# xmengli/H-DenseUNet

Measured on AMD Instinct MI355X. Metric: CT slices/sec fwd+bwd (2D 512^2), higher is better.
Workload: dtype bf16

## Files before the change

### h-denseunet_amd/csrc/conv_common.h

```cpp
#pragma once
#include "hdu_platform.h"

struct ConvK {
  const void* x;
  const void* skip;
  const void* w;
  void* y;
  const float* pro_a;
  const float* pro_b;
  const float* bias;
  const float* epi_a;
  const float* epi_b;
  int epi_relu;
  long long ldx, ldskip, ldy;
  long long M;
  int N, Di, Hi, Wi, Cin;
  int De, He, We;
  int ud, uh, uw;
  int KD, KH, KW, sd, sh, sw, pd, ph, pw;
  int Do, Ho, Wo, Cout;
  int Ktot;
  unsigned div_wo_mul, div_wo_shr, div_ho_mul, div_ho_shr, div_do_mul, div_do_shr;
  unsigned spread_h, spread_d;
  unsigned div_cin_mul, div_cin_shr, div_kw_mul, div_kw_shr, div_kh_mul, div_kh_shr;
  unsigned x_bytes, w_bytes;
  unsigned sk_div_mul, sk_div_shr;
  int pro_relu, accumulate;
  float drop_scale;
  unsigned drop_thresh;
  unsigned drop_seed;
  const unsigned* drop_seed_dev;
  int xcd_swizzle;
  int wg_gx, wg_gy, wg_gz;
  int debug_flags;
  int vec_out;
  int f32_split;
  float* stats_partial;
  const float* stats_shift;
  int stats_slots;
  const void* bnb_u; long long bnb_ldu;
  const float* bnb_a; const float* bnb_b; const float* bnb_mean; const float* bnb_rstd;
  float* bnb_partial; int bnb_slots; int bnb_relu;
  float* sk_ws;
  unsigned* sk_cnt;
  long long M_layer;
};

__device__ __forceinline__ unsigned hdu_fastdiv(unsigned n, unsigned mul, unsigned shr) {
  return mul == 0u ? n : (unsigned)(((unsigned long long)n * mul) >> 32) >> shr;
}

__device__ __forceinline__ void hdu_k_state(const ConvK& p, int k, int& c, int& kd, int& kh, int& kw, int& tap_i) {
  const unsigned tap = hdu_fastdiv((unsigned)k, p.div_cin_mul, p.div_cin_shr);
  tap_i = (int)tap;
  c = k - (int)tap * p.Cin;
  const unsigned t = hdu_fastdiv(tap, p.div_kw_mul, p.div_kw_shr);
  kw = (int)(tap - t * (unsigned)p.KW);
  const unsigned d = hdu_fastdiv(t, p.div_kh_mul, p.div_kh_shr);
  kh = (int)(t - d * (unsigned)p.KH);
  kd = (int)d;
}

__device__ __forceinline__ unsigned hdu_bit_range(int lo, int hi) {
  return (hi >= 32 ? 0xffffffffu : (1u << hi) - 1u) & ~((1u << lo) - 1u);
}

__device__ __forceinline__ unsigned hdu_tap_range_mask(int i0, int K, int E) {
  const int lo = i0 < 0 ? -i0 : 0;
  const int hi = E - i0 < K ? E - i0 : K;
  return hi > lo ? (hi >= 32 ? 0xffffffffu : (1u << hi) - 1u) & ~((1u << lo) - 1u) : 0u;
}

template <bool FAST>
__device__ __forceinline__ void hdu_row_state(const ConvK& p, unsigned m, bool pointwise, int& rn, int& rid, int& rih, int& riw,
                                              int& rpix, unsigned& rmask) {
  rmask = 0u;
  if (FAST && pointwise) {
// ... 55 lines not shown
```

### h-denseunet_amd/csrc/conv_halo_wide.hip

```cpp
#include "conv_common.h"
#include "hdu_host.h"

typedef float f32x16 __attribute__((ext_vector_type(16)));

__device__ __forceinline__ f32x16 hdu_mfma_32x32x16_bf16(u32x4 a, u32x4 b, f32x16 c) {
#ifdef HDU_EMU
  return hipemu_mfma_32x32x16_bf16(__builtin_bit_cast(hipemu_u16x8, a), __builtin_bit_cast(hipemu_u16x8, b), c);
#else
  return __builtin_amdgcn_mfma_f32_32x32x16_bf16(__builtin_bit_cast(hdu_bf16x8, a), __builtin_bit_cast(hdu_bf16x8, b), c, 0, 0, 0);
#endif
}

template <int N> __device__ __forceinline__ void hw_wait_vmcnt() {
  static_assert(N >= 0 && N < 64, "vmcnt immediate");
#ifndef HDU_EMU
  asm volatile("s_waitcnt vmcnt(%0)" ::"i"(N) : "memory");
#endif
}

template <int TH_, int NT_, int WAVES_M_, int WAVES_N_, int NS_> struct HaloWide {
  static constexpr int TH = TH_, NT = NT_, WAVES_M = WAVES_M_, WAVES_N = WAVES_N_, NS = NS_;
  static constexpr int NW = WAVES_M * WAVES_N, NTHR = NW * 64;
  static constexpr int TW = 32, HC = TW + 2, HR = TH + 2, HP = HR * HC;
  static constexpr int BN = NT * 32, BM = TH * TW;
  static constexpr int XI = (HP * 2 + 63) / 64;
  static constexpr int WI = (BN * 18 + 63) / 64;
  static constexpr int LPW = (XI + WI + NW - 1) / NW;
  static constexpr int STAGE = LPW * NW * 1024;
  static constexpr int XBYTES = XI * 1024;
  static constexpr int ROWB = BN * 2 + 16;
  static constexpr int SMEM = NS * STAGE > BM * ROWB ? NS * STAGE : BM * ROWB;
  static constexpr int MT = TH / WAVES_M, NTW = NT / WAVES_N;
  static_assert(TH % WAVES_M == 0 && NT % WAVES_N == 0, "wave layout");
  static_assert(SMEM <= 160 * 1024, "LDS");
  static_assert((NS - 2) * LPW < 64, "vmcnt");
};

template <typename C, typename RowValid>
__device__ __forceinline__ void hw_epilogue_stats(const ConvK& p, const char* smem, int n0, int tid, unsigned slot, RowValid valid) {
  constexpr int NCC = C::BN / 8, CPI = C::NTHR / 16;
  float* dst = p.stats_partial + (long long)(slot % (unsigned)p.stats_slots) * 2 * p.Cout;
  const int rl = tid & 15;
#pragma unroll 1
  for (int it = 0; it < (NCC + CPI - 1) / CPI; ++it) {
    const int cc = (tid >> 4) + it * CPI;
    const int nbase = n0 + cc * 8;
    const bool col = cc < NCC && nbase < p.Cout;
    const int ccq = col ? cc : 0, nc = col ? nbase : 0;
    float s1[8], s2[8], sh[8];
#pragma unroll
    for (int j = 0; j < 8; j += 4) {
      const f32x4 v4 = *(const f32x4*)(p.stats_shift + nc + j);
      sh[j] = v4[0]; sh[j + 1] = v4[1]; sh[j + 2] = v4[2]; sh[j + 3] = v4[3];
    }
#pragma unroll
    for (int j = 0; j < 8; ++j) { s1[j] = 0.f; s2[j] = 0.f; }
#pragma unroll 1
    for (int q0 = 0; q0 < C::BM / 16; q0 += 8) {
      u32x4 rv[8];
#pragma unroll
      for (int q = 0; q < 8; ++q) rv[q] = *(const u32x4*)(smem + (rl + (q0 + q) * 16) * C::ROWB + ccq * 16);
#pragma unroll
      for (int q = 0; q < 8; ++q) {
        const float keep = (col && valid(rl + (q0 + q) * 16)) ? 1.f : 0.f;
        float f[8];
        Chunk<bf16_t>::unpack(rv[q], f);
#pragma unroll
        for (int j = 0; j < 8; ++j) { const float d = (f[j] - sh[j]) * keep; s1[j] += d; s2[j] += d * d; }
      }
    }
#pragma unroll
    for (int j = 0; j < 8; ++j) { s1[j] = hdu_row16_sum(s1[j]); s2[j] = hdu_row16_sum(s2[j]); }
    float mine = 0.f;
#pragma unroll
    for (int j = 0; j < 8; ++j) {
      mine = rl == j ? s1[j] : mine;
      mine = rl == 8 + j ? s2[j] : mine;
    }
    if (col) atomicAdd(dst + (rl < 8 ? 0 : p.Cout) + nbase + (rl & 7), mine);
  }
}

template <typename C>
__device__ __forceinline__ void hw_epilogue(const ConvK& p, f32x16 (&acc)[C::MT][C::NTW], char* smem, long long mplane, int y0, int x0,
                                            int n0, int wm, int wn, int lane, int tid, unsigned slot) {
  typedef bf16_t T;
  constexpr int BN = C::BN, BM = C::BM, NTHR = C::NTHR, ROWB = C::ROWB, MT = C::MT, NTW = C::NTW;
  const int l31 = lane & 31, lh = lane >> 5;
  hw_wait_vmcnt<0>();
  __syncthreads();
  const unsigned dseed = p.drop_seed + (p.drop_seed_dev ? *p.drop_seed_dev : 0u);
  const bool has_bias = p.bias != nullptr, drop = p.drop_scale != 0.f, has_epi = p.epi_a != nullptr;
#pragma unroll
  for (int j = 0; j < NTW; ++j) {
    f32x4 bias_v[4], epa_v[4], epb_v[4];
#pragma unroll
    for (int g = 0; g < 4; ++g) {
      const int nn = n0 + (wn * NTW + j) * 32 + 8 * g + 4 * lh;
      const int nc = nn < p.Cout ? nn : 0;
      bias_v[g] = has_bias ? *(const f32x4*)(p.bias + nc) : f32x4{0.f, 0.f, 0.f, 0.f};
      epa_v[g] = has_epi ? *(const f32x4*)(p.epi_a + nc) : f32x4{1.f, 1.f, 1.f, 1.f};
      epb_v[g] = has_epi ? *(const f32x4*)(p.epi_b + nc) : f32x4{0.f, 0.f, 0.f, 0.f};
    }
#pragma unroll
    for (int i = 0; i < MT; ++i) {
      const int trow = wm * MT + i;
      const int row = trow * 32 + l31;
      const long long m = (mplane + y0 + trow) * p.Wo + x0 + l31;
#pragma unroll
      for (int g = 0; g < 4; ++g) {
        const int col = (wn * NTW + j) * 32 + 8 * g + 4 * lh;
        const int nn = n0 + col;
        float v[4] = {acc[i][j][4 * g], acc[i][j][4 * g + 1], acc[i][j][4 * g + 2], acc[i][j][4 * g + 3]};
        if (has_bias) {
#pragma unroll
          for (int r = 0; r < 4; ++r) v[r] += bias_v[g][r];
        }
        if (drop) {
#pragma unroll
          for (int r = 0; r < 4; ++r) {
            const unsigned h = hdu_hash32((unsigned long long)m * (unsigned)p.Cout + (unsigned)(nn + r), dseed);
            v[r] = h < p.drop_thresh ? v[r] * p.drop_scale : 0.f;
          }
        }
        if (has_epi) {
#pragma unroll
          for (int r = 0; r < 4; ++r) {
            v[r] = epa_v[g][r] * v[r] + epb_v[g][r];
            if (p.epi_relu) v[r] = v[r] > 0.f ? v[r] : 0.f;
          }
        }
        Chunk<T>::store4((T*)(smem + row * ROWB) + col, v);
      }
    }
  }
  __syncthreads();
  T* __restrict__ yp = (T*)p.y;
  constexpr int NCC = BN / 8;
  constexpr int NIT = (BM * NCC + NTHR - 1) / NTHR;
  auto out_ptr = [&](int q, bool& ok) -> T* {
    const int row = q / NCC, cc = q - row * NCC;
    const int oy = y0 + (row >> 5), ox = x0 + (row & 31);
    const int nn = n0 + cc * 8;
    ok = q < BM * NCC && oy < p.Ho && ox < p.Wo && nn < p.Cout;
    return ok ? yp + ((mplane + oy) * p.Wo + ox) * p.ldy + nn : yp;
  };
  if (p.accumulate) {
#pragma unroll 1
    for (int it0 = 0; it0 < NIT; it0 += 4) {
      u32x4 old[4];
      T* dst[4];
      bool ok[4];
#pragma unroll
      for (int u = 0; u < 4; ++u) {
        dst[u] = out_ptr(tid + (it0 + u) * NTHR, ok[u]);
        ok[u] = ok[u] && it0 + u < NIT;
        old[u] = *(const u32x4*)dst[u];
      }
#pragma unroll
      for (int u = 0; u < 4; ++u) {
        if (!ok[u]) continue;
        const int q = tid + (it0 + u) * NTHR;
        const int row = q / NCC, cc = q - row * NCC;
        float f[8], g[8];
        Chunk<T>::unpack(*(const u32x4*)(smem + row * ROWB + cc * 16), f);
        Chunk<T>::unpack(old[u], g);
#pragma unroll
        for (int jj = 0; jj < 8; ++jj) f[jj] += g[jj];
        *(u32x4*)dst[u] = Chunk<T>::pack(f);
      }
    }
  } else {
#pragma unroll
    for (int it = 0; it < NIT; ++it) {
      const int q = tid + it * NTHR;
      bool ok;
      T* dst = out_ptr(q, ok);
      if (!ok) continue;
      const int row = q / NCC, cc = q - row * NCC;
      *(u32x4*)dst = *(const u32x4*)(smem + row * ROWB + cc * 16);
// ... 130 lines not shown
      }
#pragma unroll
      for (int j = 0; j < NTW; ++j) bf[j] = *(const u32x4*)(Xs + wrow_off[j] + tap * 32);
#pragma unroll
      for (int i = 0; i < MT; ++i)
#pragma unroll
        for (int j = 0; j < NTW; ++j) acc[i][j] = hdu_mfma_32x32x16_bf16(bf[j], af[i], acc[i][j]);
#pragma unroll
      for (int u = 0; u < PER_TAP; ++u)
        if (tap * PER_TAP + u < LPW) issue_piece(nxsrd, nwoff, nc0, nbase, tap * PER_TAP + u, more);
    }
    slot = slot == NS - 1 ? 0 : slot + 1;
  }

  const long long mplane = ((long long)n * p.Do + od) * p.Ho;
  hw_epilogue<C>(p, acc, smem, mplane, y0, x0, n0, wm, wn, lane, tid, blockIdx.x);
}

struct StemCfg {
  static constexpr int TH = 16, NT = 3, WAVES_M = 8, WAVES_N = 1, NS = 4;
  static constexpr int NW = 8, NTHR = 512, TW = 32;
  static constexpr int BN = 96, BM = TH * TW;
  static constexpr int SEG = 70;
  static constexpr int XSLOTS = TH * SEG;
  static constexpr int XI = (XSLOTS + 63) / 64;
  static constexpr int WSLOTS = BN * 9;
  static constexpr int WI = (WSLOTS + 63) / 64;
  static constexpr int LPW = (XI + WI + NW - 1) / NW;
  static constexpr int STAGE = LPW * NW * 1024;
  static constexpr int XBYTES = XI * 1024;
  static constexpr int ROWB = BN * 2 + 16;
  static constexpr int SMEM = NS * STAGE > BM * ROWB ? NS * STAGE : BM * ROWB;
  static constexpr int MT = 2, NTW = 3;
  static_assert(SMEM <= 160 * 1024, "LDS");
};

__global__ __launch_bounds__(StemCfg::NTHR) void conv_stem_s2_kernel(ConvK p, int tiles_x, int tiles_y, int ngroups) {
  typedef StemCfg C;
  typedef bf16_t T;
  constexpr int NW = C::NW, NS = C::NS, XI = C::XI, WI = C::WI, LPW = C::LPW, STAGE = C::STAGE, XBYTES = C::XBYTES, SEG = C::SEG;
  constexpr int MT = C::MT, NTW = C::NTW, BN = C::BN;
  __shared__ __attribute__((aligned(16))) char smem[C::SMEM];
  const int tid = threadIdx.x;
  const int lane = tid & 63;
#ifdef HDU_EMU
  const int wave = tid >> 6;
#else
  const int wave = __builtin_amdgcn_readfirstlane(tid >> 6);
#endif
  const T* __restrict__ xp = (const T*)p.x;
  unsigned t = (p.xcd_swizzle & 1) ? xcd_tile_index(blockIdx.x, gridDim.x) : blockIdx.x;
  const int ng = (int)(t % (unsigned)ngroups); t /= (unsigned)ngroups;
  const int od = (int)(t % (unsigned)p.Do); t /= (unsigned)p.Do;
  const int txi = (int)(t % (unsigned)tiles_x); t /= (unsigned)tiles_x;
  const int tyi = (int)(t % (unsigned)tiles_y);
  const int n = (int)(t / (unsigned)tiles_y);
  const int y0 = tyi * C::TH, x0 = txi * C::TW;
  const int n0 = ng * BN;

  unsigned roff[LPW];
  int riy[LPW];
#pragma unroll
  for (int j = 0; j < LPW; ++j) {
    const int jj = j * NW + wave;
    riy[j] = -(1 << 28);
    if (jj < XI) {
// ... 307 lines not shown
  if (force == 1 || !hw_shape_ok(k, dtype)) return 0;
  if (force >= 2) return force - 1 <= NCFG ? force - 1 : 0;
  if (k.Cin < 32 || k.Cout < 48 || k.We < 24) return 0;
  const double scale = (double)k.M_layer / (double)k.M;
  constexpr int NC = 7;
  const int th[NC] = {8, 16, 16, 8, 8, 16, 16}, nt[NC] = {4, 2, 3, 2, 3, 4, 2}, occ[NC] = {1, 1, 1, 2, 2, 1, 2};
  const double busy[NC] = {0.60, 0.68, 0.68, 0.58, 0.58, 0.74, 0.76};
  const double nst = (double)((k.Cin + 15) / 16) * k.KD;
  bool deep16 = false;
  if (nst >= 24. && !(g_tuning[HDU_TUNE_DEBUG] & 1024))
    for (int c = 0; c < NC; ++c)
      if (th[c] == 16 && (double)k.N * k.Do * ((k.He + 15) / 16) * ((k.We + 31) / 32) * scale * (double)((k.Cout + nt[c] * 32 - 1) / (nt[c] * 32)) >= 128.)
        deep16 = true;
  int best = 0;
  double best_cost = 0., best_wgs = 0.;
  for (int c = 0; c < NC; ++c) {
    if (deep16 && th[c] == 8) continue;
    if (c == 6 && (g_tuning[HDU_TUNE_DEBUG] & 512)) continue;
    const int bn = nt[c] * 32;
    const double wgs = (double)k.N * k.Do * ((k.He + th[c] - 1) / th[c]) * ((k.We + 31) / 32) * scale * (double)((k.Cout + bn - 1) / bn);
    const double load = __builtin_ceil(wgs / 256.0);
    const double work = (double)th[c] * nt[c];
    const double main_ = nst * work / ((c == 6 && load < 4.) ? 0.50 : busy[c]);
    const double fixed = 40.0 + work;
    const double cost = load * main_ + __builtin_ceil(load / occ[c]) * fixed * ((occ[c] == 2 && load >= 2.) ? 0.3 : 1.0);
    if (best == 0 || cost < best_cost) { best = c + 1; best_cost = cost; best_wgs = wgs; }
  }
  if (best_wgs < 128.) return 0;
  if (k.Cout < 64 && best_wgs < 1024.) return 0;
  return best;
}

static bool stem_geom_ok(const ConvK& k, int dtype) {
  if (g_tuning[HDU_TUNE_HALO_WIDE] == 1 || dtype != HDU_BF16) return false;
  if (k.bnb_u != nullptr || k.pro_a != nullptr || k.skip != nullptr || !k.vec_out || (k.ud | k.uh | k.uw) != 0) return false;
  if (k.KH != 7 || k.KW != 7 || k.sh != 2 || k.sw != 2 || k.ph != 3 || k.pw != 3 || k.Cin != 8) return false;
  if (!((k.KD == 1 && k.sd == 1 && k.pd == 0) || (k.KD == 7 && k.sd == 2 && k.pd >= 0 && k.pd <= 3))) return false;
  if (k.Ho != (k.Hi + 6 - 7) / 2 + 1 || k.Wo != (k.Wi + 6 - 7) / 2 + 1 || k.Do != (k.Di + 2 * k.pd - k.KD) / k.sd + 1) return false;
  if (k.Cout % 8) return false;
  return (long long)k.Hi * k.Wi * k.ldx * 2 < (1ll << 31);
}

static bool stem_ok(const ConvK& k, int dtype) {
  if (!stem_geom_ok(k, dtype)) return false;
  const long long wgs = (long long)k.N * k.Do * ((k.Ho + 15) / 16) * ((k.Wo + 31) / 32) * ((k.Cout + 95) / 96);
  if (wgs >= (1ll << 31)) return false;
  if (g_tuning[HDU_TUNE_HALO_WIDE] >= 2) return true;
  return k.Wo >= 24 && wgs * k.M_layer / k.M >= 128;
}

static void stem_launch(const ConvK& k, hipStream_t s) {
  const int tiles_x = (k.Wo + 31) / 32, tiles_y = (k.Ho + 15) / 16, ngroups = (k.Cout + 95) / 96;
  const unsigned grid = (unsigned)((long long)k.N * k.Do * tiles_x * tiles_y * ngroups);
  HDU_LAUNCH(conv_stem_s2_kernel, dim3(grid), dim3(StemCfg::NTHR), 0, s, k, tiles_x, tiles_y, ngroups);
}

bool hdu_stem_wgrad_taken(const ConvK& k, int dtype) {
  return stem_geom_ok(k, dtype) && k.ldy % 8 == 0 && (long long)k.Ho * k.Wo * k.ldy * 2 < (1ll << 31) &&
         (long long)k.Cout * k.KD * 49 * 8 < (1ll << 31);
}

bool hdu_stem_wgrad_launch(const ConvK& k, int dtype, float* dw, hipStream_t s) {
  if (!hdu_stem_wgrad_taken(k, dtype)) return false;
  const int tiles_x = (k.Wo + 31) / 32, tiles_y = (k.Ho + 3) / 4, ngroups = (k.Cout + 95) / 96;
  const long long tiles = (long long)k.N * k.Do * tiles_x * tiles_y;
  long long nsplit = 512 / ((long long)k.KD * ngroups);
  if (nsplit > tiles / 32) nsplit = tiles / 32;
// ... 30 lines not shown
```

### h-denseunet_amd/csrc/conv_igemm.hip

```cpp
#include "conv_common.h"
#include "../../include/hdu.h"

template <typename T, int BM, int BN> struct BnbGeom {
  static constexpr int CH = Chunk<T>::CH;
  static constexpr int NCC = BN / CH;
  static constexpr int NCCP = NCC <= 4 ? 4 : (NCC <= 8 ? 8 : (NCC <= 16 ? 16 : 32));
  static constexpr int RSTEP = 256 / NCCP;
  static constexpr int IT = (BM + RSTEP - 1) / RSTEP;
  static constexpr bool EARLY = IT <= 8;
  static_assert(NCC <= 32, "tile shape");
};

template <bool SPLIT, typename T, int BM, int BN, int WAVES_M, int WAVES_N>
__device__ __forceinline__ void conv_igemm_body(const ConvK& p, char* smem) {
  constexpr int CH = Chunk<T>::CH;
  constexpr int BK = 8 * CH;
  constexpr int A_IT = BM / 32;
  constexpr int B_IT = (BN + 31) / 32;
  constexpr int WM = BM / WAVES_M;
  constexpr int WN = BN / WAVES_N;
  constexpr int TM = WM / 16;
  constexpr int TN = WN / 16;
  constexpr int STAGE = (BM + BN) * 128;
  static_assert(WAVES_M * WAVES_N == 4, "4 waves");
// ... 2802 lines not shown
    k->x_bytes = xb > 0 && xb < (1ll << 32) ? (unsigned)xb : 0u;
    if (g_tuning[HDU_TUNE_DEBUG] & 16) k->x_bytes = 0u;
    if (!wgrad && wb >= (1ll << 32)) return hdu_set_error(HDU_ERR_ARG, "conv: filter larger than 4 GiB");
    k->w_bytes = (unsigned)wb;
  }
  k->pro_relu = d->pro_relu; k->accumulate = d->accumulate;
  if (d->drop_keep > 0.f && d->drop_keep < 1.f) {
    k->drop_scale = 1.f / d->drop_keep;
    k->drop_thresh = (unsigned)((double)d->drop_keep * 4294967296.0);
  } else {
    k->drop_scale = 0.f;
    k->drop_thresh = 0xffffffffu;
  }
  k->drop_seed = d->drop_seed;
  k->drop_seed_dev = d->drop_seed_dev;
  k->stats_partial = wgrad ? nullptr : d->stats_partial;
  k->stats_shift = d->stats_shift;
  k->stats_slots = d->stats_slots;
  if (k->stats_partial && (!k->stats_shift || k->stats_slots <= 0 || d->accumulate))
    return hdu_set_error(HDU_ERR_ARG, "conv: epilogue statistics need stats_shift, stats_slots > 0 and accumulate == 0");
  k->bnb_u = wgrad ? nullptr : d->bnb_u; k->bnb_ldu = d->bnb_ldu;
  k->bnb_a = d->bnb_a; k->bnb_b = d->bnb_b; k->bnb_mean = d->bnb_mean; k->bnb_rstd = d->bnb_rstd;
  k->bnb_relu = d->bnb_relu; k->bnb_partial = d->bnb_partial; k->bnb_slots = d->bnb_slots;
  if (k->bnb_u) {
    if (!k->bnb_a || !k->bnb_b || (uintptr_t)k->bnb_u % 16 || k->bnb_ldu % ch || d->pro_a || d->skip || d->bias ||
        d->stats_partial || (d->drop_keep > 0.f && d->drop_keep < 1.f))
      return hdu_set_error(HDU_ERR_ARG, "conv: the fused BN backward needs bnb_a/bnb_b, a 16-byte addressable bnb_u and a plain data-gradient launch (no prologue / skip / bias / dropout / statistics)");
    if (k->bnb_partial && (!k->bnb_mean || !k->bnb_rstd || k->bnb_slots <= 0))
      return hdu_set_error(HDU_ERR_ARG, "conv: bnb_partial needs bnb_mean, bnb_rstd and bnb_slots > 0");
  }
  if (((uintptr_t)k->bias | (uintptr_t)k->epi_a | (uintptr_t)k->epi_b | (uintptr_t)(k->stats_partial ? k->stats_shift : nullptr) |
       (uintptr_t)k->bnb_a | (uintptr_t)k->bnb_b | (uintptr_t)k->bnb_mean | (uintptr_t)k->bnb_rstd) & 15)
    return hdu_set_error(HDU_ERR_ARG, "conv: bias / epi_* / stats_shift / bnb_* vectors must be 16-byte aligned");
  k->M_layer = d->layer_rows > 0 ? d->layer_rows : k->M;
  k->sk_ws = wgrad ? nullptr : (float*)d->splitk_ws;
  k->sk_cnt = wgrad ? nullptr : d->splitk_counters;
  if (k->sk_ws && ((uintptr_t)k->sk_ws % 16 || !k->sk_cnt))
    return hdu_set_error(HDU_ERR_ARG, "conv: splitk_ws must be 16-byte aligned and come with splitk_counters");
  k->xcd_swizzle = g_tuning[HDU_TUNE_XCD_SWIZZLE];
  k->vec_out = 1;
  k->debug_flags = g_tuning[HDU_TUNE_DEBUG];
  k->f32_split = (d->dtype == HDU_F32 && g_tuning[HDU_TUNE_F32_SPLIT]) ? 1 : 0;
  if (!wgrad && d->y && (d->Cout % ch || d->ldy % ch || (uintptr_t)d->y % 16))
    return hdu_set_error(HDU_ERR_ARG, "conv: Cout / output pixel stride must be multiples of the 16-byte chunk and y 16-byte aligned");
  return 0;
}

static bool igemm_fast_ok(const ConvK& k) {
  if (g_tuning[HDU_TUNE_NO_FAST]) return false;
  if ((k.ud | k.uh | k.uw) != 0 || k.KD * k.KH * k.KW > 32) return false;
  const long long span = ((long long)k.N * k.De * k.He * k.We + (long long)k.He * k.We * 8) * k.ldx;
  return span < (1ll << 31) && k.x_bytes != 0;
}

static bool conv_pointwise(const ConvK& k) {
  return k.KD * k.KH * k.KW == 1 && k.sd == 1 && k.sh == 1 && k.sw == 1 && (k.pd | k.ph | k.pw) == 0 && (k.ud | k.uh | k.uw) == 0;
}

static bool igemm_pro_dma_ok(const ConvK& k) {
  return k.pro_a != nullptr && k.skip == nullptr && k.vec_out && k.bnb_u == nullptr && conv_pointwise(k) && k.Cin <= HDU_PRO_CMAX &&
         k.Do == k.De && k.Ho == k.He && k.Wo == k.We && igemm_fast_ok(k) && !g_tuning[HDU_TUNE_NO_PRO_DMA] &&
         ((uintptr_t)k.pro_a % 16 == 0) && ((uintptr_t)k.pro_b % 16 == 0);
}

static int ring_wgs_per_cu(int bm, bool bf16) { return (bm == 64 && bf16) ? 2 : 1; }

// ... 221 lines not shown
  const unsigned ny = (unsigned)((k.Cout + BN - 1) / BN);
  long long splits = target / (long long)ny;
  if (splits < 1) splits = 1;
  const long long tiles = (k.M + 63) / 64;
  if (splits > tiles) splits = tiles;
  const long long rows = ((tiles + splits - 1) / splits) * 64;
  const unsigned gx = (unsigned)((k.M + rows - 1) / rows);
  if (k.bnb_u != nullptr) {
    if (k.Ktot == 192) HDU_LAUNCH((conv_pw_bstat_kernel<3, BN, true, NSA>), dim3(gx, ny), dim3(256), 0, s, k, (int)rows);
    else HDU_LAUNCH((conv_pw_bstat_kernel<2, BN, true, NSA>), dim3(gx, ny), dim3(256), 0, s, k, (int)rows);
    return;
  }
  if (k.Ktot == 192) HDU_LAUNCH((conv_pw_bstat_kernel<3, BN, false, NSA>), dim3(gx, ny), dim3(256), 0, s, k, (int)rows);
  else HDU_LAUNCH((conv_pw_bstat_kernel<2, BN, false, NSA>), dim3(gx, ny), dim3(256), 0, s, k, (int)rows);
}

static int pw_bstat_form(const ConvK& k) {
  const int f = g_tuning[HDU_TUNE_PW_BSTAT_FORM];
  if (f == 1 || f == 2) return f;
  return k.bnb_u != nullptr ? 2 : 1;
}

static void launch_pw_bstat(const ConvK& k, hipStream_t s) {
  const int wgs = g_tuning[HDU_TUNE_PW_BSTAT_WGS];
  if (pw_bstat_form(k) == 2) launch_pw_bstat_form<64, 2>(k, wgs > 0 ? wgs : 512, s);
  else launch_pw_bstat_form<128, 3>(k, wgs > 0 ? wgs : 256, s);
}

extern "C" int hdu_conv_fprop(const hdu_conv_desc* d, void* stream) {
  ConvK k;
  if (int e = fill_convk(d, &k, false)) return e;
  if (!d->y) return hdu_set_error(HDU_ERR_ARG, "conv_fprop: null output");
  if (k.M == 0) return 0;
  if (pw_bstat_ok(k, d->dtype)) {
    launch_pw_bstat(k, (hipStream_t)stream);
    return hdu_check_launch("conv_fprop(pointwise, filter-stationary)");
  }
  if (hdu_halo_wide_launch(k, d->dtype, (hipStream_t)stream)) return hdu_check_launch("conv_fprop(halo, wide)");
  if (fprop_halo_ok(k, d->dtype)) {
    switch (choose_halo_bn(k)) {
      case 96: launch_halo_fprop<96>(k, (hipStream_t)stream); break;
      case 64: launch_halo_fprop<64>(k, (hipStream_t)stream); break;
      case 48: launch_halo_fprop<48>(k, (hipStream_t)stream); break;
      default: launch_halo_fprop<32>(k, (hipStream_t)stream); break;
    }
    return hdu_check_launch("conv_fprop(halo)");
  }
  if (d->dtype == HDU_BF16) dispatch_igemm<bf16_t>(k, d->splitk_ws_bytes, (hipStream_t)stream);
  else dispatch_igemm<float>(k, d->splitk_ws_bytes, (hipStream_t)stream);
  return hdu_check_launch("conv_fprop");
}

extern "C" size_t hdu_conv_splitk_ws_bytes(const hdu_conv_desc* d) {
  ConvK k;
  if (fill_convk(d, &k, false)) return 0;
  if (k.M == 0 || pw_bstat_ok(k, d->dtype) || hdu_halo_wide_taken(k, d->dtype) || fprop_halo_ok(k, d->dtype) || (k.pro_a != nullptr && !igemm_pro_dma_ok(k)) || k.skip != nullptr) return 0;
  int bm, bn;
  choose_igemm(k, &bm, &bn);
  if (bm == 128 && igemm_pers_ok(k, bn)) return 0;
  const long long nblk = ((k.M + bm - 1) / bm) * ((k.Cout + bn - 1) / bn);
  const long long nblk_layer = ((k.M_layer + bm - 1) / bm) * ((k.Cout + bn - 1) / bn);
  const int stage = (bm + ((bn + 31) / 32) * 32) * 128;
  const int nsd = stage * 6 <= 160 * 1024 ? 6 : 4;
  if (!igemm_ring_ok(nblk_layer, k.Ktot, stage, nsd)) return 0;
  const int bk = d->dtype == HDU_BF16 ? 64 : 32;
  size_t need;
// ... 378 lines not shown
```

### h-denseunet_amd/engine.py

```python
import ctypes
import math
import os
from collections import OrderedDict

import numpy as np
import torch

from . import ops
from . import shard as _sh
from .lib import HDU_BF16, HDU_F32


class Param:
    __slots__ = ("layer", "idx", "kind", "keras_shape", "shape", "trainable", "init", "offset", "numel", "ctx", "meta")

    def __init__(self, ctx, layer, idx, kind, keras_shape, shape, trainable, init, meta=None):
        self.ctx, self.layer, self.idx, self.kind = ctx, layer, idx, kind
        self.keras_shape, self.shape, self.trainable, self.init = tuple(keras_shape), tuple(shape), trainable, init
        self.numel = int(np.prod(shape))
        self.offset = None
        self.meta = meta or {}

    @property
    def data(self):
# ... 97 lines not shown


class Ctx:

    def __init__(self, dtype, batch_shape):
        self.dtype = dtype
        self.ch = ops.CHUNK[dtype]
        self.params = []
        self.by_layer = OrderedDict()
        self.layer_kind = OrderedDict()
        self.fwd = []
        self.bwd = _BwdList(self)
        self.vars = []
        self.learning_phase = 1
        self.pass_id = 0
        self.P = self.G = self.V = None
        self.n_trainable = 0
        self.convs = []
        self.bns = []
        self._fold_plans = {}
        self._prefolded_phase = None
        self.prefolded_pass = -1
        self.batch_fold = os.environ.get("HDU_BATCH_FOLD", "1") == "1"
        self.defer_bnb_finalize = os.environ.get("HDU_DEFER_BNB_FINALIZE", "1") == "1"
        self._bnb_deferred, self._bnb_plan = [], None
        self._pending_fin = None
        self.merge_fin_correct = os.environ.get("HDU_MERGE_FIN_CORRECT", "1") == "1"
        self.absorb_stats = os.environ.get("HDU_ABSORB_STATS", "1") == "1"
        self.bn_bwd_fused = os.environ.get("HDU_BN_BWD_FUSED", "1") == "1"
        self.fuse_bn_bwd_mode = int(os.environ.get("HDU_FUSE_BN_BWD", "1"))
        self.fuse_bn_bwd = self.fuse_bn_bwd_mode > 0
        self.fuse_bn_bwd_pw = os.environ.get("HDU_FUSE_BN_BWD_PW", "1") == "1"
        self.bnb_sums_epilogue = os.environ.get("HDU_BNB_SUMS_EPILOGUE", "1") == "1"
        self.head_dz_fused = os.environ.get("HDU_HEAD_DZ_FUSED", "1") == "1"
        self.bias_sums_in_apply = os.environ.get("HDU_BIAS_SUMS_IN_APPLY", "1") == "1"
        self._csum_deferred, self._csum_plan = [], None
        self.fuse_bn_bwd_now = False
        self.bnb_sinks = []
        self.bnb_acc = None
        self.corr_acc = None
        self._corr_total = 0
        self._scratch = {}
        self.ws_bytes = 1 << 16
        self.ws = None
        self.dev = ops.device()
        self.seed_dev = torch.zeros(1, dtype=torch.int32, device=self.dev)
        self.drop_layers = 0
        self.dropout_enabled = True
        self.grad_enabled = True
        self.fuse_bn_epilogue = os.environ.get("HDU_FUSE_BN_EPILOGUE", "1") == "1"
        self.fuse_bn_epilogue_train = os.environ.get("HDU_FUSE_BN_EPILOGUE_TRAIN", "1") == "1"
        self.fold_next = os.environ.get("HDU_FOLD_NEXT", "1") == "1"
        self.shard = None
        self.fuse_prologue = os.environ.get("HDU_FUSE_PROLOGUE", "0") == "1"
        self.fuse_pw = os.environ.get("HDU_FUSE_PW", "1") == "1"
        self.batch_wgrad = os.environ.get("HDU_BATCH_WGRAD", "1") == "1"
        self.wgrad_plan = None
        self.split_wgrad = os.environ.get("HDU_F32_SPLIT_WGRAD", "1") == "1"
        self._split_plan = None
        self._split_now = False
        self.epilogue_stats = os.environ.get("HDU_EPILOGUE_STATS", "1") == "1"
        self.stats_sinks = []
        self.stat_roots = []
        self.stats_acc = None
        self.finalized = False
        self.arena = None
# ... 590 lines not shown
                             and stride == (1, 1, 1) and pad == (0, 0, 0) and up == (0, 0, 0) and cin_p <= ops.PRO_CMAX)
        if self.pw_fused:
            pass
        elif halo:
            self.xin = ctx.new_var(xa.N, xa.D + 2 * halo, xa.H, xa.W, cin_p)
            plane = xa.H * xa.W * cin_p
            self.xin_interior = ops.Act(self.xin.act.buf, halo * plane, xa.N, xa.D, xa.H, xa.W, cin_p, cin_p, dt)
            self._halo_tmp = ctx.scratch("halo_tmp", 1, 2 * halo, xa.H, xa.W, cin_p)
        elif (bn is not None or skip is not None) and not ctx.fuse_prologue:
            if skip is not None:
                self.xin = ctx.new_var(xa.N, De, He, We, cin_p)
                self.conv_up = (0, 0, 0)
            else:
                self.xin = ctx.new_var(xa.N, xa.D, xa.H, xa.W, cin_p)
        st = getattr(bn, "stats_src", None) if bn is not None else None
        if (st is not None and self.xin is not None and not halo and st.producer is not None and st.absorber is None
                and x.root is st.var.root and bn.C == x.C and x.c0 == (0 if bn is st.fold_next else st.var.c0)):
            st.absorber = self
        self.need_input_grad = need_input_grad
        self.epi_consumer = None
        self.epi_producer = None
        if (producer is not None and ctx.fuse_bn_epilogue and bn is not None and self.xin is not None and not halo
                and skip is None and up == (0, 0, 0) and x is producer.out and x.root is x and producer.epi_consumer is None):
            self.epi_producer = producer
            producer.epi_consumer = self
        self.strided = stride != (1, 1, 1)
        pw_stream = bool(ctx.fuse_bn_bwd_pw and dt == HDU_BF16 and K == (1, 1, 1) and pad == (0, 0, 0) and cout_p in (128, 192)
                         and cin_p >= 256 and xa.M >= 64)
        self.bnb_fused = bool(ctx.fuse_bn_bwd and need_input_grad and bn is not None and up == (0, 0, 0) and skip is None
                              and not halo and stride == (1, 1, 1) and not ctx.fuse_prologue and x.root.drop is None
                              and (ctx.fuse_bn_bwd_mode >= 2 or bn.mode != "batch" or pw_stream))
        self.bnb_off = None
        self._sums_kernel_ok = None
        self._s2 = None
        self._s2_ok = (os.environ.get("HDU_STRIDE2_DGRAD", "1") == "1" and all(v in (1, 2) for v in stride)
                       and xa.D % stride[0] == 0 and xa.H % stride[1] == 0 and xa.W % stride[2] == 0 and up == (0, 0, 0)
                       and bn is None and skip is None and not halo)
        self.need_dgrad_filter = need_input_grad and not self.strided
        self.wf_off = self.wd_off = None
        ctx.convs.append(self)
        if bn is not None:
            ctx.need_ws(xa.M, xa.C)
        ctx.need_ws(out.act.M, cout_p)
        if need_input_grad:
            if bn is not None or up != (0, 0, 0) or halo:
                self._dxe = ctx.scratch("dxe", xa.N, De, He, We, cin_p)
            if (bn is not None or halo) and up != (0, 0, 0):
                self._dz = ctx.scratch("dz", xa.N, xa.D + 2 * halo, xa.H, xa.W, cin_p)
        ctx.fwd.append(self.forward)
        ctx.bwd.append(self.backward)

    def bind(self):
        ctx = self.ctx
        esz = ctx.Wc.element_size()
        if ctx.dtype == HDU_F32:
            self.wf_ptr = ctypes.c_void_p(self.kernel.data.data_ptr())
        else:
            self.wf_ptr = ctypes.c_void_p(ctx.Wc.data_ptr() + self.wf_off * esz)
        self.wd_ptr = ctypes.c_void_p(ctx.Wc.data_ptr() + self.wd_off * esz) if self.need_dgrad_filter else None
        x, out = self.x.act, self.out.act
        pro = (self.bn.a, self.bn.b) if self.bn is not None else None
        relu = self.bn.relu if self.bn is not None else False
        skip = self.skip.act if self.skip is not None else None
        up = self.up
        if self.xin is not None:
            x, pro, relu, skip, up = self.xin.act, None, False, None, self.conv_up
# ... 103 lines not shown
            if self.bias is not None:
                self._bias_grad(dy)
        if not self.need_input_grad:
            return
        K, pad = self.K, self.pad
        if self.halo:
            return self._backward_halo(dy)
        if self.bnb_fused and ctx.fuse_bn_bwd_now:
            return self._backward_fused_bn(dy)
        if self._head_dz_fused():
            return self.bn.backward(self.x, dy, pw=(self.wd_ptr, self.filters))
        De, He, We = x.D << self.up[0], x.H << self.up[1], x.W << self.up[2]
        direct = self.bn is None and self.up == (0, 0, 0)
        sums_ready = False
        skip_first = self.skip is not None and self.skip.root.needs_grad and not self.skip.root.written \
            and self.skip.c0 == 0
        if direct:
            tgt, acc = self.x.grad, self.x.grad_mode()
        elif skip_first:
            tgt, acc = self.skip.grad, self.skip.grad_mode()
        else:
            tgt, acc = self._dxe(), False
        if self.strided:
            tgt_act = ops.Act(tgt.buf, tgt.off, x.N, x.D, x.H, x.W, x.C, tgt.ld, tgt.dtype)
            if self._s2 is not None:
                self._s2.run(tgt_act, accumulate=acc)
            else:
                d = ctx.conv_desc(tgt_act, self.wf_ptr, dy, K, self.stride, pad, accumulate=acc)
                ops.conv_dgrad_strided(d)
        else:
            d = ctx.conv_desc(dy, self.wd_ptr, ops.Act(tgt.buf, tgt.off, x.N, De, He, We, x.C, tgt.ld, tgt.dtype), K,
                              (1, 1, 1), (K[0] - 1 - pad[0], K[1] - 1 - pad[1], K[2] - 1 - pad[2]), accumulate=acc)
            sums_ready = self._epilogue_sums(d)
            ops.conv_fprop(d)
        if self.skip is not None and self.skip.root.needs_grad and not skip_first:
            ops.upsample_bwd(tgt, self.skip.grad, (0, 0, 0), accumulate=self.skip.grad_mode())
        if direct:
            return
        dz = tgt
        if self.up != (0, 0, 0):
            if self.bn is None:
                ops.upsample_bwd(tgt, self.x.grad, self.up, accumulate=self.x.grad_mode())
                return
            dz = self._dz()
            ops.upsample_bwd(tgt, dz, self.up)
        if self.bn is not None:
            self.bn.backward(self.x, dz, sums_ready=sums_ready)
        else:
            ops.upsample_bwd(dz, self.x.grad, (0, 0, 0), accumulate=self.x.grad_mode())

    def _bias_grad(self, dy):
        ctx, r = self.ctx, self.out.root
        if self.csum is not None and r.csum_pass == ctx.pass_id and r.n_writes == 1:
            ctx._csum_deferred.append((id(self), (self.csum, self.CSUM_SLOTS, self.cout_p, self.bias.grad)))
        else:
            ops.colsum(dy, self.bias.grad, ctx.ws)

    def _head_dz_fused(self):
        ctx, bn = self.ctx, self.bn
        return bool(ctx.head_dz_fused and bn is not None and self.K == (1, 1, 1) and self.stride == (1, 1, 1)
                    and self.pad == (0, 0, 0) and self.up == (0, 0, 0) and self.skip is None and not self.halo
                    and self.cout_p == ops.CHUNK[ctx.dtype] and self.filters <= 4 and self.wd_ptr is not None
                    and self.wd_ptr.value % 16 == 0 and self.out.grad.ptr.value % 16 == 0
                    and not (ctx.shard is not None and ctx.shard.world > 1) and bn.takes_epilogue_sums(self.x))

    def _epilogue_sums(self, d):
        ctx, bn = self.ctx, self.bn
        if not (ctx.bnb_sums_epilogue and bn is not None and self.up == (0, 0, 0) and self.skip is None and not self.halo
                and self.x.root.drop is None and ctx.bnb_fusable() and bn.BSUM_SLOTS <= 32):
            return False
        if self._sums_kernel_ok is None:
            name = ops.conv_kernel_name(d, 0)
            self._sums_kernel_ok = name.startswith("conv_igemm_ring_kernel") or name.startswith("conv_igemm_dma_kernel")
        if not self._sums_kernel_ok or not bn.takes_epilogue_sums(self.x):
            return False
        x = self.x.act
        d.bnb_u, d.bnb_ldu = x.ptr, x.ld
        d.bnb_a, d.bnb_b = bn.a.data_ptr(), bn.b.data_ptr()
        d.bnb_relu = (1 if bn.relu else 0) | 4
        d.bnb_mean, d.bnb_rstd = bn.mean_used.data_ptr(), bn.rstd.data_ptr()
        d.bnb_partial, d.bnb_slots = bn.bsum.data_ptr(), bn.BSUM_SLOTS
        return True


def _conv_backward_fused_bn(self, dy):
    ctx, bn, xv = self.ctx, self.bn, self.x
    x = xv.act
    K, pad = self.K, self.pad
    acc = xv.grad_mode()
    tgt = xv.grad
    d = ctx.conv_desc(dy, self.wd_ptr, ops.Act(tgt.buf, tgt.off, x.N, x.D, x.H, x.W, x.C, tgt.ld, tgt.dtype), K, (1, 1, 1),
                      (K[0] - 1 - pad[0], K[1] - 1 - pad[1], K[2] - 1 - pad[2]), accumulate=acc)
    d.bnb_u, d.bnb_ldu = x.ptr, x.ld
    d.bnb_a, d.bnb_b, d.bnb_relu = bn.a.data_ptr(), bn.b.data_ptr(), 1 if bn.relu else 0
    if self.epi_producer is not None and self.epi_active():
        d.bnb_u, d.bnb_ldu = self.xin.act.ptr, self.xin.act.ld
        d.bnb_relu |= 2
# ... 282 lines not shown
```

### h-denseunet_amd/lib.py

```python
import ctypes
import os

_HERE = os.path.dirname(os.path.abspath(__file__))
_ROOT = os.path.dirname(_HERE)

HDU_BF16 = 0
HDU_F32 = 1

c_int, c_i64, c_f, c_p, c_u32, c_sz = (ctypes.c_int, ctypes.c_int64, ctypes.c_float, ctypes.c_void_p,
                                       ctypes.c_uint32, ctypes.c_size_t)


class ConvDesc(ctypes.Structure):
    _fields_ = [
        ("dtype", c_int),
        ("x", c_p), ("ldx", c_i64),
        ("N", c_int), ("Di", c_int), ("Hi", c_int), ("Wi", c_int), ("Cin", c_int),
        ("ud", c_int), ("uh", c_int), ("uw", c_int),
        ("skip", c_p), ("ldskip", c_i64),
        ("pro_a", c_p), ("pro_b", c_p), ("pro_relu", c_int),
        ("w", c_p),
        ("KD", c_int), ("KH", c_int), ("KW", c_int),
        ("sd", c_int), ("sh", c_int), ("sw", c_int),
        ("pd", c_int), ("ph", c_int), ("pw", c_int),
        ("y", c_p), ("ldy", c_i64),
        ("Do", c_int), ("Ho", c_int), ("Wo", c_int), ("Cout", c_int),
        ("bias", c_p),
        ("epi_a", c_p), ("epi_b", c_p), ("epi_relu", c_int),
        ("accumulate", c_int),
        ("drop_keep", c_f),
        ("drop_seed", c_u32),
        ("drop_seed_dev", c_p),
        ("stats_partial", c_p),
        ("stats_shift", c_p),
        ("stats_slots", c_int),
        ("bnb_u", c_p), ("bnb_ldu", c_i64),
        ("bnb_a", c_p), ("bnb_b", c_p), ("bnb_mean", c_p), ("bnb_rstd", c_p),
        ("bnb_relu", c_int),
        ("bnb_partial", c_p), ("bnb_slots", c_int),
        ("splitk_ws", c_p),
        ("splitk_ws_bytes", c_sz),
        ("splitk_counters", c_p),
        ("layer_rows", ctypes.c_int64),
    ]


class PrepEntry(ctypes.Structure):
    _fields_ = [("master_off", c_i64), ("w_f_off", c_i64), ("w_d_off", c_i64), ("tile_begin", c_i64),
                ("Cout", ctypes.c_int32), ("T", ctypes.c_int32), ("Cin", ctypes.c_int32), ("pad_", ctypes.c_int32)]


class AugSample(ctypes.Structure):
    _fields_ = [("img_off", c_i64), ("vrows", ctypes.c_int32), ("vcols", ctypes.c_int32), ("vslices", ctypes.c_int32),
                ("a0", ctypes.c_int32), ("b0", ctypes.c_int32), ("c0", ctypes.c_int32), ("crop", ctypes.c_int32),
                ("flip", ctypes.c_int32)]


class ZeroEntry(ctypes.Structure):
    _fields_ = [("ptr", c_p), ("bytes", ctypes.c_uint64), ("block_begin", ctypes.c_uint32), ("pad_", ctypes.c_uint32),
                ("src", c_p)]


class BnBwdEntry(ctypes.Structure):
    _fields_ = [("partial", c_p), ("slots", ctypes.c_int32), ("C", ctypes.c_int32), ("gamma", c_p), ("beta", c_p),
                ("sgamma", c_p), ("dgamma", c_p), ("dbeta", c_p), ("dsgamma", c_p), ("dsbeta", c_p)]


class ColsumEntry(ctypes.Structure):
    _fields_ = [("partial", c_p), ("out", c_p), ("slots", ctypes.c_int32), ("C", ctypes.c_int32)]


class BnStatsFold(ctypes.Structure):
    _fields_ = [("partial", c_p), ("slots", ctypes.c_int32), ("Cseg", ctypes.c_int32), ("seg_c0", ctypes.c_int32),
                ("pad_", ctypes.c_int32), ("M", c_i64), ("shift", c_p), ("mean", c_p), ("var", c_p), ("gamma", c_p),
                ("beta", c_p), ("sgamma", c_p), ("sbeta", c_p), ("eps", c_f), ("momentum", c_f), ("a", c_p), ("b", c_p),
                ("rstd", c_p), ("mov_mean", c_p), ("mov_var", c_p)]
# ... 104 lines not shown
                                             c_p, c_p]),
    "hdu_pp_threshold": (c_int, [c_p, c_p, c_int, c_int, c_int, c_int, c_int, c_int, ctypes.c_double, ctypes.c_double, c_p, c_p, c_p]),
    "hdu_pp_dilate": (c_int, [c_p, c_int, c_int, c_int, c_p, c_p]),
    "hdu_pp_label": (c_int, [c_p, c_int, c_int, c_int, c_int, c_int, c_p, c_p]),
    "hdu_pp_largest": (c_int, [c_p, c_int, c_int, c_int, c_p, c_p, c_p, c_p, c_p]),
    "hdu_pp_fill_holes": (c_int, [c_p, c_int, c_int, c_int, c_p, c_p, c_p, c_p]),
    "hdu_pp_bbox": (c_int, [c_p, c_int, c_int, c_int, c_p, c_p]),
    "hdu_pp_merge": (c_int, [c_int, c_p, c_p, c_i64, c_p, c_p]),
    "hdu_zero_regions": (c_int, [c_p, c_int, c_u32, c_p, c_u32, c_p]),
    "hdu_zero": (c_int, [c_p, ctypes.c_uint64, c_p]),
    "hdu_split3_entry_fill": (c_int, [c_p, c_p, c_i64, c_i64, c_int, c_p, c_p, c_int, c_int, c_p, c_u32, ctypes.POINTER(c_u32)]),
    "hdu_split3_batched": (c_int, [c_p, c_int, c_u32, c_int, c_p]),
    "hdu_profile_begin": (c_int, [c_int]),
    "hdu_profile_count": (c_int, []),
    "hdu_profile_end": (c_int, []),
    "hdu_profile_get": (c_int, [c_int, ctypes.c_char_p, c_sz, ctypes.POINTER(c_f)]),
    "hdu_comm_unique_id": (c_int, [c_p]),
    "hdu_comm_init": (c_int, [ctypes.POINTER(c_p), c_int, c_int, c_p]),
    "hdu_comm_destroy": (c_int, [c_p]),
    "hdu_comm_allreduce_f32": (c_int, [c_p, c_p, c_i64, c_p]),
    "hdu_comm_sendrecv": (c_int, [c_p, c_int, c_p, c_p, c_int, c_p, c_p, c_sz, c_p]),
}

EXPORTS = tuple(_SIGS.keys())

_lib = None
_backend = None


class HduError(RuntimeError):
    pass


ABI_VERSION = 11


def product_library_path():
    return os.path.join(_HERE, "libhdu.so")


def _bind(path):
    import torch
    lib = ctypes.CDLL(path)
    for name, (res, args) in _SIGS.items():
        fn = getattr(lib, name)
        fn.restype = res
        fn.argtypes = args
    if lib.hdu_abi_version() != ABI_VERSION or lib.hdu_sizeof_conv_desc() != ctypes.sizeof(ConvDesc):
        raise HduError("%s has ABI version %d / hdu_conv_desc of %d bytes, this binding expects %d / %d -- rebuild it "
                       "(python -c 'import __graft_entry__ as g; g.build()')" %
                       (path, lib.hdu_abi_version(), lib.hdu_sizeof_conv_desc(), ABI_VERSION, ctypes.sizeof(ConvDesc)))
    return lib


def _apply_env_tuning(lib):
    if "HDU_DMA_STAGES" in os.environ:
        lib.hdu_set_tuning(0, int(os.environ["HDU_DMA_STAGES"]))
    if "HDU_SPLITK" in os.environ:
        lib.hdu_set_tuning(13, int(os.environ["HDU_SPLITK"]))
    if "HDU_BM64_MAX_M" in os.environ:
        lib.hdu_set_tuning(18, int(os.environ["HDU_BM64_MAX_M"]))
    if "HDU_SPLITK_TARGET" in os.environ:
        lib.hdu_set_tuning(16, int(os.environ["HDU_SPLITK_TARGET"]))
    if "HDU_SPLITK_MIN_STEPS" in os.environ:
        lib.hdu_set_tuning(17, int(os.environ["HDU_SPLITK_MIN_STEPS"]))
    if "HDU_HALO_MIN_TILES" in os.environ:
        lib.hdu_set_tuning(15, int(os.environ["HDU_HALO_MIN_TILES"]))
# ... 167 lines not shown
```

### include/hdu.h

```cpp
#ifndef HDU_H_
#define HDU_H_

#include <stddef.h>
#include <stdint.h>

#ifdef __cplusplus
extern "C" {
#endif

#define HDU_BF16 0
#define HDU_F32 1

#define HDU_OK 0
#define HDU_ERR_ARG (-1)
#define HDU_ERR_LAUNCH (-2)
#define HDU_ERR_WORKSPACE (-3)

const char* hdu_last_error(void);
const char* hdu_backend(void);
#define HDU_ABI_VERSION 11
int hdu_abi_version(void);
size_t hdu_sizeof_conv_desc(void);
int hdu_profile_begin(int max_records);
int hdu_profile_count(void);
int hdu_profile_end(void);
int hdu_profile_get(int i, char* name_buf, size_t buflen, float* ms);
#define HDU_TUNE_DMA_STAGES 0
#define HDU_TUNE_HALO_TARGET_WGS 7
#define HDU_TUNE_MAX_BN 6
#define HDU_TUNE_NO_FAST 5
#define HDU_TUNE_DEBUG 4
#define HDU_TUNE_XCD_SWIZZLE 3
#define HDU_TUNE_RED_WGS 11
#define HDU_TUNE_ROW_WGS 12
#define HDU_TUNE_NO_HALO_FPROP 9
#define HDU_TUNE_NO_HALO 8
#define HDU_TUNE_WGRAD_TARGET_WGS 2
#define HDU_TUNE_SPLITK 13
#define HDU_TUNE_BM64_MAX_M 18
#define HDU_TUNE_SPLITK_TARGET 16
#define HDU_TUNE_SPLITK_MIN_STEPS 17
#define HDU_TUNE_HALO_MIN_TILES 15
#define HDU_TUNE_RING_MIN_K 14
#define HDU_TUNE_WGRAD_MIN_STEPS 1
#define HDU_TUNE_NO_PW_BSTAT 19
#define HDU_TUNE_PW_BSTAT_WGS 20
#define HDU_TUNE_PW_BSTAT_FORM 30
#define HDU_TUNE_NO_PRO_DMA 22
#define HDU_TUNE_PERS 23
#define HDU_TUNE_NO_PW_BSTAT_BNB 26
#define HDU_TUNE_PERS_MIN_ITEMS 24
#define HDU_TUNE_HALO_MIN_W 28
#define HDU_TUNE_F32_SPLIT 27
// ... 2 lines not shown
#define HDU_TUNE_WGRAD_NCT 21
int hdu_set_tuning(int key, int value);

typedef struct hdu_conv_desc {
  int dtype;
  const void* x;      int64_t ldx;
  int N, Di, Hi, Wi, Cin;
  int ud, uh, uw;
  const void* skip;   int64_t ldskip;
  const float* pro_a; const float* pro_b; int pro_relu;
  const void* w;
  int KD, KH, KW;
  int sd, sh, sw;
  int pd, ph, pw;
  void* y;            int64_t ldy;
  int Do, Ho, Wo, Cout;
  const float* bias;
  const float* epi_a; const float* epi_b; int epi_relu;
  int accumulate;
  float drop_keep;
  uint32_t drop_seed;
  const uint32_t* drop_seed_dev;
  float* stats_partial;
  const float* stats_shift;
  int stats_slots;
  const void* bnb_u;  int64_t bnb_ldu;
  const float* bnb_a; const float* bnb_b; const float* bnb_mean; const float* bnb_rstd;
  int bnb_relu;
  float* bnb_partial; int bnb_slots;
  void* splitk_ws;
  size_t splitk_ws_bytes;
  uint32_t* splitk_counters;
  int64_t layer_rows;
} hdu_conv_desc;

int hdu_bn_bwd_finalize(const float* partial, int slots, int64_t M, int C, int batch_stats, const float* gamma,
                        const float* beta, const float* sgamma, const float* mean, const float* rstd, float* dgamma,
                        float* dbeta, float* dsgamma, float* dsbeta, float* corr3, float* corr4, void* stream);

typedef struct hdu_bnbwd_entry {
  const float* partial;
  int32_t slots, C;
  const float* gamma; const float* beta; const float* sgamma;
  float* dgamma; float* dbeta; float* dsgamma; float* dsbeta;
} hdu_bnbwd_entry;
int hdu_bn_bwd_finalize_batched(const hdu_bnbwd_entry* table, const uint32_t* begins, int n, uint32_t total_blocks, void* stream);

typedef struct hdu_colsum_entry {
  const float* partial;
  float* out;
  int32_t slots, C;
} hdu_colsum_entry;
int hdu_colsum_fold_batched(const hdu_colsum_entry* table, const uint32_t* begins, int n, uint32_t total_blocks, void* stream);

int hdu_bn_bwd_correct(int dtype, const void* u, int64_t ldu, int64_t M, int C, const float* corr3, const float* corr4,
                       void* du, int64_t lddu, void* stream);
int hdu_bn_bwd_finalize_correct(int dtype, const float* partial, int slots, int64_t M, int C, const float* gamma, const float* beta,
                                const float* sgamma, const float* mean, const float* rstd, float* dgamma, float* dbeta,
                                float* dsgamma, float* dsbeta, float* corr3, float* corr4, int cs0, int Cc, const void* u,
                                int64_t ldu, void* du, int64_t lddu, void* stream);

size_t hdu_conv_splitk_ws_bytes(const hdu_conv_desc* d);

int hdu_conv_fprop(const hdu_conv_desc* d, void* stream);

int hdu_conv_wgrad(const hdu_conv_desc* d, float* dw, void* stream);
// ... 238 lines not shown
```

Before: 546.3.

## Fuse upsample backward 2x2 sum-pooling into halo-wide dgrad conv epilogue

Adds a down-sampled output to the halo-wide conv epilogue. It sums each 2x2 block of the output tile, already staged in LDS, and writes it to a second buffer, optionally accumulating or skipping the full-resolution store. The engine uses this for the dgrad of layers with (0,1,1) upsampling, so a separate upsample_bwd pass and the full-resolution gradient write plus re-read are no longer needed. It costs an ABI bump, extra epilogue work, and restrictions: even Ho/Wo and halo-wide kernels only.

```diff
diff --git a/h-denseunet_amd/csrc/conv_common.h b/h-denseunet_amd/csrc/conv_common.h
--- a/h-denseunet_amd/csrc/conv_common.h
+++ b/h-denseunet_amd/csrc/conv_common.h
@@ -43,6 +43,8 @@
   float* bnb_partial; int bnb_slots; int bnb_relu;
   float* sk_ws;
   unsigned* sk_cnt;
+  void* y_ds; long long ldy_ds;
+  int ds_accumulate, ds_only;
   long long M_layer;
 };
 
diff --git a/h-denseunet_amd/csrc/conv_halo_wide.hip b/h-denseunet_amd/csrc/conv_halo_wide.hip
--- a/h-denseunet_amd/csrc/conv_halo_wide.hip
+++ b/h-denseunet_amd/csrc/conv_halo_wide.hip
@@ -31,7 +31,9 @@
   static constexpr int ROWB = BN * 2 + 16;
   static constexpr int SMEM = NS * STAGE > BM * ROWB ? NS * STAGE : BM * ROWB;
   static constexpr int MT = TH / WAVES_M, NTW = NT / WAVES_N;
+  static constexpr bool DS = true;
   static_assert(TH % WAVES_M == 0 && NT % WAVES_N == 0, "wave layout");
+  static_assert(TH % 2 == 0 && TW % 2 == 0, "a 2 x 2 block of the output grid lies inside one tile");
   static_assert(SMEM <= 160 * 1024, "LDS");
   static_assert((NS - 2) * LPW < 64, "vmcnt");
 };
@@ -82,6 +84,40 @@
 }
 
 template <typename C>
+__device__ __forceinline__ void hw_epilogue_ds(const ConvK& p, const char* smem, long long mplane, int y0, int x0, int n0, int tid) {
+  typedef bf16_t T;
+  constexpr int NCC = C::BN / 8, NQ = (C::BM / 4) * NCC, NIT = (NQ + C::NTHR - 1) / C::NTHR, ROWB = C::ROWB;
+  T* __restrict__ zp = (T*)p.y_ds;
+  const long long mplane_ds = mplane >> 1;
+  const int Wd = p.Wo >> 1;
+#pragma unroll
+  for (int it = 0; it < NIT; ++it) {
+    const int q = tid + it * C::NTHR;
+    const int blk = q / NCC, cc = q - blk * NCC;
+    const int ty = (blk >> 4) * 2, tx = (blk & 15) * 2;
+    const int oy = y0 + ty, ox = x0 + tx, nn = n0 + cc * 8;
+    if (q >= NQ || oy >= p.Ho || ox >= p.Wo || nn >= p.Cout) continue;
+    const char* src = smem + (ty * 32 + tx) * ROWB + cc * 16;
+    float s[8], f[8];
+#pragma unroll
+    for (int j = 0; j < 8; ++j) s[j] = 0.f;
+#pragma unroll
+    for (int b = 0; b < 4; ++b) {
+      Chunk<T>::unpack(*(const u32x4*)(src + ((b >> 1) * 32 + (b & 1)) * ROWB), f);
+#pragma unroll
+      for (int j = 0; j < 8; ++j) s[j] += f[j];
+    }
+    T* dst = zp + ((mplane_ds + (oy >> 1)) * Wd + (ox >> 1)) * p.ldy_ds + nn;
+    if (p.ds_accumulate) {
+      Chunk<T>::unpack(*(const u32x4*)dst, f);
+#pragma unroll
+      for (int j = 0; j < 8; ++j) s[j] += f[j];
+    }
+    *(u32x4*)dst = Chunk<T>::pack(s);
+  }
+}
+
+template <typename C>
 __device__ __forceinline__ void hw_epilogue(const ConvK& p, f32x16 (&acc)[C::MT][C::NTW], char* smem, long long mplane, int y0, int x0,
                                             int n0, int wm, int wn, int lane, int tid, unsigned slot) {
   typedef bf16_t T;
@@ -135,6 +171,9 @@
     }
   }
   __syncthreads();
+  if constexpr (C::DS) {
+    if (p.y_ds) hw_epilogue_ds<C>(p, smem, mplane, y0, x0, n0, tid);
+  }
   T* __restrict__ yp = (T*)p.y;
   constexpr int NCC = BN / 8;
   constexpr int NIT = (BM * NCC + NTHR - 1) / NTHR;
@@ -145,7 +184,8 @@
     ok = q < BM * NCC && oy < p.Ho && ox < p.Wo && nn < p.Cout;
     return ok ? yp + ((mplane + oy) * p.Wo + ox) * p.ldy + nn : yp;
   };
-  if (p.accumulate) {
+  if (C::DS && p.ds_only) {
+  } else if (p.accumulate) {
 #pragma unroll 1
     for (int it0 = 0; it0 < NIT; it0 += 4) {
       u32x4 old[4];
@@ -342,6 +382,7 @@
   static constexpr int ROWB = BN * 2 + 16;
   static constexpr int SMEM = NS * STAGE > BM * ROWB ? NS * STAGE : BM * ROWB;
   static constexpr int MT = 2, NTW = 3;
+  static constexpr bool DS = false;
   static_assert(SMEM <= 160 * 1024, "LDS");
 };
 
@@ -715,7 +756,7 @@
 }
 
 static bool stem_geom_ok(const ConvK& k, int dtype) {
-  if (g_tuning[HDU_TUNE_HALO_WIDE] == 1 || dtype != HDU_BF16) return false;
+  if (g_tuning[HDU_TUNE_HALO_WIDE] == 1 || dtype != HDU_BF16 || k.y_ds != nullptr) return false;
   if (k.bnb_u != nullptr || k.pro_a != nullptr || k.skip != nullptr || !k.vec_out || (k.ud | k.uh | k.uw) != 0) return false;
   if (k.KH != 7 || k.KW != 7 || k.sh != 2 || k.sw != 2 || k.ph != 3 || k.pw != 3 || k.Cin != 8) return false;
   if (!((k.KD == 1 && k.sd == 1 && k.pd == 0) || (k.KD == 7 && k.sd == 2 && k.pd >= 0 && k.pd <= 3))) return false;
diff --git a/h-denseunet_amd/csrc/conv_igemm.hip b/h-denseunet_amd/csrc/conv_igemm.hip
--- a/h-denseunet_amd/csrc/conv_igemm.hip
+++ b/h-denseunet_amd/csrc/conv_igemm.hip
@@ -2858,6 +2858,17 @@
   if (((uintptr_t)k->bias | (uintptr_t)k->epi_a | (uintptr_t)k->epi_b | (uintptr_t)(k->stats_partial ? k->stats_shift : nullptr) |
        (uintptr_t)k->bnb_a | (uintptr_t)k->bnb_b | (uintptr_t)k->bnb_mean | (uintptr_t)k->bnb_rstd) & 15)
     return hdu_set_error(HDU_ERR_ARG, "conv: bias / epi_* / stats_shift / bnb_* vectors must be 16-byte aligned");
+  k->y_ds = wgrad ? nullptr : d->y_ds; k->ldy_ds = d->ldy_ds;
+  k->ds_accumulate = d->ds_accumulate; k->ds_only = d->ds_only;
+  if (k->y_ds) {
+    if ((d->Ho | d->Wo) & 1) return hdu_set_error(HDU_ERR_ARG, "conv: the down-sampled output needs even Ho and Wo");
+    if ((uintptr_t)k->y_ds % 16 || k->ldy_ds % ch || k->ldy_ds < d->Cout)
+      return hdu_set_error(HDU_ERR_ARG, "conv: y_ds must be 16-byte aligned and ldy_ds a multiple of the 16-byte chunk >= Cout");
+    if (d->accumulate) return hdu_set_error(HDU_ERR_ARG, "conv: the down-sampled output excludes accumulate (it sums what a plain store holds)");
+    if (exact_grid) return hdu_set_error(HDU_ERR_ARG, "conv: the down-sampled output is a halo-wide hdu_conv_fprop epilogue only");
+  } else if (!wgrad && (d->ds_only || d->ds_accumulate)) {
+    return hdu_set_error(HDU_ERR_ARG, "conv: ds_only / ds_accumulate without y_ds");
+  }
   k->M_layer = d->layer_rows > 0 ? d->layer_rows : k->M;
   k->sk_ws = wgrad ? nullptr : (float*)d->splitk_ws;
   k->sk_cnt = wgrad ? nullptr : d->splitk_counters;
@@ -3145,6 +3156,8 @@
   if (int e = fill_convk(d, &k, false)) return e;
   if (!d->y) return hdu_set_error(HDU_ERR_ARG, "conv_fprop: null output");
   if (k.M == 0) return 0;
+  if (k.y_ds && !hdu_halo_wide_taken(k, d->dtype))
+    return hdu_set_error(HDU_ERR_ARG, "conv_fprop: y_ds needs a launch that a halo-wide configuration takes");
   if (pw_bstat_ok(k, d->dtype)) {
     launch_pw_bstat(k, (hipStream_t)stream);
     return hdu_check_launch("conv_fprop(pointwise, filter-stationary)");
diff --git a/h-denseunet_amd/engine.py b/h-denseunet_amd/engine.py
--- a/h-denseunet_amd/engine.py
+++ b/h-denseunet_amd/engine.py
@@ -153,6 +153,7 @@
         self.fuse_bn_bwd = self.fuse_bn_bwd_mode > 0
         self.fuse_bn_bwd_pw = os.environ.get("HDU_FUSE_BN_BWD_PW", "1") == "1"
         self.bnb_sums_epilogue = os.environ.get("HDU_BNB_SUMS_EPILOGUE", "1") == "1"
+        self.ups_bwd_epilogue = os.environ.get("HDU_UPS_BWD_EPILOGUE", "1") == "1"
         self.head_dz_fused = os.environ.get("HDU_HEAD_DZ_FUSED", "1") == "1"
         self.bias_sums_in_apply = os.environ.get("HDU_BIAS_SUMS_IN_APPLY", "1") == "1"
         self._csum_deferred, self._csum_plan = [], None
@@ -809,6 +810,7 @@
                               and (ctx.fuse_bn_bwd_mode >= 2 or bn.mode != "batch" or pw_stream))
         self.bnb_off = None
         self._sums_kernel_ok = None
+        self._ups_kernel_ok = None
         self._s2 = None
         self._s2_ok = (os.environ.get("HDU_STRIDE2_DGRAD", "1") == "1" and all(v in (1, 2) for v in stride)
                        and xa.D % stride[0] == 0 and xa.H % stride[1] == 0 and xa.W % stride[2] == 0 and up == (0, 0, 0)
@@ -978,7 +980,12 @@
             d = ctx.conv_desc(dy, self.wd_ptr, ops.Act(tgt.buf, tgt.off, x.N, De, He, We, x.C, tgt.ld, tgt.dtype), K,
                               (1, 1, 1), (K[0] - 1 - pad[0], K[1] - 1 - pad[1], K[2] - 1 - pad[2]), accumulate=acc)
             sums_ready = self._epilogue_sums(d)
+            ups_dz = self._ups_epilogue(d, direct, skip_first, acc)
             ops.conv_fprop(d)
+            if ups_dz is not None:
+                if self.bn is not None:
+                    self.bn.backward(self.x, ups_dz, sums_ready=sums_ready)
+                return
         if self.skip is not None and self.skip.root.needs_grad and not skip_first:
             ops.upsample_bwd(tgt, self.skip.grad, (0, 0, 0), accumulate=self.skip.grad_mode())
         if direct:
@@ -1009,6 +1016,27 @@
                     and self.cout_p == ops.CHUNK[ctx.dtype] and self.filters <= 4 and self.wd_ptr is not None
                     and self.wd_ptr.value % 16 == 0 and self.out.grad.ptr.value % 16 == 0
                     and not (ctx.shard is not None and ctx.shard.world > 1) and bn.takes_epilogue_sums(self.x))
+
+    def _ups_epilogue(self, d, direct, skip_first, acc):
+        ctx = self.ctx
+        if not ctx.ups_bwd_epilogue or direct or self.up != (0, 1, 1) or self.halo or ctx.dtype != HDU_BF16:
+            return None
+        if self.skip is not None and self.skip.root.needs_grad and not skip_first:
+            return None
+        if skip_first and acc:
+            return None
+        if self._ups_kernel_ok is None:
+            self._ups_kernel_ok = ops.conv_kernel_name(d, 0).startswith("conv_halo_wide_kernel")
+        if not self._ups_kernel_ok:
+            return None
+        if self.bn is not None:
+            dz, dacc = self._dz(), False
+        else:
+            dz, dacc = self.x.grad, self.x.grad_mode()
+        d.y_ds, d.ldy_ds = dz.ptr, dz.ld
+        d.ds_accumulate = 1 if dacc else 0
+        d.ds_only = 0 if skip_first else 1
+        return dz
 
     def _epilogue_sums(self, d):
         ctx, bn = self.ctx, self.bn
diff --git a/h-denseunet_amd/lib.py b/h-denseunet_amd/lib.py
--- a/h-denseunet_amd/lib.py
+++ b/h-denseunet_amd/lib.py
@@ -42,6 +42,9 @@
         ("splitk_ws_bytes", c_sz),
         ("splitk_counters", c_p),
         ("layer_rows", ctypes.c_int64),
+        ("y_ds", c_p), ("ldy_ds", c_i64),
+        ("ds_accumulate", c_int),
+        ("ds_only", c_int),
     ]
 
 
@@ -212,7 +215,7 @@
     pass
 
 
-ABI_VERSION = 11
+ABI_VERSION = 12
 
 
 def product_library_path():
diff --git a/include/hdu.h b/include/hdu.h
--- a/include/hdu.h
+++ b/include/hdu.h
@@ -18,7 +18,7 @@
 
 const char* hdu_last_error(void);
 const char* hdu_backend(void);
-#define HDU_ABI_VERSION 11
+#define HDU_ABI_VERSION 12
 int hdu_abi_version(void);
 size_t hdu_sizeof_conv_desc(void);
 int hdu_profile_begin(int max_records);
@@ -87,6 +87,9 @@
   size_t splitk_ws_bytes;
   uint32_t* splitk_counters;
   int64_t layer_rows;
+  void* y_ds;         int64_t ldy_ds;
+  int ds_accumulate;
+  int ds_only;
 } hdu_conv_desc;
 
 int hdu_bn_bwd_finalize(const float* partial, int slots, int64_t M, int C, int batch_stats, const float* gamma,
```

Result: faster. 551.8, median of 6 (+1.0%).
